# feixue94/sfd2

Hardware: AMD Instinct MI355X
Metric: images/sec extract+match (1600x1200, n4096) (higher is better)
Workload: dtype f16c

## Files before the change

### sfd2_amd/csrc/conv1x1_kernels.hip

```cpp
#include "sfd2_internal.h"
#include <stdlib.h>
#include <algorithm>

#define NT1 512
#define GPX 64
#define NST 4
#define STAGE_BYTES (GPX * 512)

typedef __attribute__((address_space(3))) void lds_void_t;
typedef const __attribute__((address_space(1))) void gbl_void_t;

__device__ __forceinline__ h4_t c1_cvt4(float a, float b, float c, float d)
{
    h4_t r;
    r[0] = (half_t)a; r[1] = (half_t)b; r[2] = (half_t)c; r[3] = (half_t)d;
    return r;
}

template <bool HAS_RES>
__global__ __launch_bounds__(NT1, 2)
void conv1x1_c256_kernel(const half_t *__restrict__ in, int npix, const half_t *__restrict__ w ,
                         const float *__restrict__ scale, const float *__restrict__ shift, int relu,
                         const half_t *__restrict__ res, half_t *__restrict__ out, int groups_per_block,
                         const half_t *__restrict__ zero_page )
{
    extern __shared__ __attribute__((aligned(16))) unsigned char smem[];
    unsigned char *Xs = smem;
    float *SS = reinterpret_cast<float *>(smem + NST * STAGE_BYTES);

    const int tid = threadIdx.x, lane = tid & 63;
    const int wave = __builtin_amdgcn_readfirstlane(tid >> 6);
    const int lrow = lane & 31, lhi = lane >> 5;
    const int cg = wave & 3, ph = wave >> 2;
    const int ngroups = (npix + GPX - 1) / GPX;
    const int g0 = blockIdx.x * groups_per_block;
    int g1 = g0 + groups_per_block;
    if (g1 > ngroups) g1 = ngroups;
    if (g0 >= g1) return;

    h8_t a[2][16];
#pragma unroll
    for (int t = 0; t < 2; ++t)
#pragma unroll
        for (int kk = 0; kk < 16; ++kk)
            a[t][kk] = *reinterpret_cast<const h8_t *>(w + (size_t)(cg * 64 + t * 32 + lrow) * 256 + kk * 16 + lhi * 8);
    for (int t = tid; t < 256; t += NT1) { SS[t] = scale[t]; SS[256 + t] = shift[t]; }

#define ISSUE_G(g_)                                                                                        \
    {                                                                                                      \
        unsigned char *st = Xs + ((g_) & (NST - 1)) * STAGE_BYTES;                                         \
        _Pragma("unroll") for (int i = 0; i < 4; ++i) {                                                    \
            const int ch = wave * 4 + i;                                                                   \
            const int p = ch * 2 + lhi;                                        \
            const long long gp = (long long)(g_)*GPX + p;                                                  \
            const half_t *src = gp < npix ? in + gp * 256 + ((lrow ^ (p & 31)) << 3) : zero_page + (lrow << 3); \
            __builtin_amdgcn_global_load_lds((gbl_void_t *)src, (lds_void_t *)(st + ch * 1024), 16, 0, 0); \
        }                                                                                                  \
    }
#define WAIT_GROUP()                                                                                       \
    asm volatile("s_waitcnt vmcnt(8) lgkmcnt(0)\n\ts_barrier" ::: "memory")

    ISSUE_G(g0)
    if (g0 + 1 < g1) { ISSUE_G(g0 + 1) }
    if (g0 + 2 < g1) { ISSUE_G(g0 + 2) }
    SFD2_BARRIER_DRAIN();

    for (int g = g0; g < g1; ++g) {
        if (g != g0) {
            if (g + 2 < g1) WAIT_GROUP(); else SFD2_BARRIER_DRAIN();
        }
        const unsigned char *st = Xs + (g & (NST - 1)) * STAGE_BYTES;
        const int p = ph * 32 + lrow;
        const long long gp = (long long)g * GPX + p;
        const bool inb = gp < npix;
        const size_t obase = (size_t)(inb ? gp : 0) * 256 + cg * 64;

        uint4 rq[2][2];
        if (HAS_RES) {
#pragma unroll
            for (int t = 0; t < 2; ++t)
#pragma unroll
                for (int m = 0; m < 2; ++m) {
                    rq[t][m] = make_uint4(0, 0, 0, 0);
                    if (inb) rq[t][m] = *reinterpret_cast<const uint4 *>(res + obase + t * 32 + 8 * (2 * m + lhi));
                }
            asm volatile("" ::: "memory");
        }
        if (g + 3 < g1) { ISSUE_G(g + 3) }

        f32x16_t acc[2];
#pragma unroll
        for (int t = 0; t < 2; ++t)
#pragma unroll
            for (int r = 0; r < 16; ++r) acc[t][r] = 0.0f;
        const unsigned char *xp = st + p * 512;
        const int sw = p & 31;
#pragma unroll
        for (int kk = 0; kk < 16; ++kk) {
            const h8_t b = *reinterpret_cast<const h8_t *>(xp + (((kk * 2 + lhi) ^ sw) << 4));
            acc[0] = __builtin_amdgcn_mfma_f32_32x32x16_f16(a[0][kk], b, acc[0], 0, 0, 0);
            acc[1] = __builtin_amdgcn_mfma_f32_32x32x16_f16(a[1][kk], b, acc[1], 0, 0, 0);
        }

#pragma unroll
        for (int t = 0; t < 2; ++t) {
            const int cl = cg * 64 + t * 32 + 4 * lhi;
#pragma unroll
            for (int m = 0; m < 2; ++m) {
                uint2 rp[2] = {make_uint2(0, 0), make_uint2(0, 0)};
                if (HAS_RES) {
                    const auto s0 = __builtin_amdgcn_permlane32_swap(rq[t][m].x, rq[t][m].z, false, false);
                    const auto s1 = __builtin_amdgcn_permlane32_swap(rq[t][m].y, rq[t][m].w, false, false);
                    rp[0] = make_uint2(s0[0], s1[0]);
                    rp[1] = make_uint2(s0[1], s1[1]);
                }
                uint2 pk[2];
#pragma unroll
                for (int j = 0; j < 2; ++j) {
                    const int q = 2 * m + j;
                    const float4 sc = sfd2_lds_f4(SS + cl + 8 * q);
                    const float4 sh = sfd2_lds_f4(SS + 256 + cl + 8 * q);
                    float v0 = acc[t][4 * q + 0] * sc.x + sh.x;
                    float v1 = acc[t][4 * q + 1] * sc.y + sh.y;
                    float v2 = acc[t][4 * q + 2] * sc.z + sh.z;
                    float v3 = acc[t][4 * q + 3] * sc.w + sh.w;
                    if (HAS_RES) {
                        h4_t r;
                        __builtin_memcpy(&r, &rp[j], 8);
                        v0 += (float)r[0]; v1 += (float)r[1]; v2 += (float)r[2]; v3 += (float)r[3];
                    }
                    if (relu) { v0 = fmaxf(v0, 0.0f); v1 = fmaxf(v1, 0.0f); v2 = fmaxf(v2, 0.0f); v3 = fmaxf(v3, 0.0f); }
                    const h4_t hv = c1_cvt4(v0, v1, v2, v3);
                    __builtin_memcpy(&pk[j], &hv, 8);
                }
                const auto t0 = __builtin_amdgcn_permlane32_swap(pk[0].x, pk[1].x, false, false);
                const auto t1 = __builtin_amdgcn_permlane32_swap(pk[0].y, pk[1].y, false, false);
                if (inb)
                    *reinterpret_cast<uint4 *>(out + obase + t * 32 + 8 * (2 * m + lhi)) = make_uint4(t0[0], t1[0], t0[1], t1[1]);
            }
        }
    }
#undef ISSUE_G
#undef WAIT_GROUP
}

void launch_conv1x1_c256(hipStream_t st, const half_t *in, int npix, const half_t *w_rowmajor, const float *scale,
                         const float *shift, int relu, const half_t *res, half_t *out, const half_t *zero_page)
{
    static bool attr_done = false;
    static int slots = 256;
    const size_t lds = (size_t)NST * STAGE_BYTES + 512 * sizeof(float);
    if (!attr_done) {
        (void)hipFuncSetAttribute(reinterpret_cast<const void *>(conv1x1_c256_kernel<true>), hipFuncAttributeMaxDynamicSharedMemorySize, (int)lds);
        (void)hipFuncSetAttribute(reinterpret_cast<const void *>(conv1x1_c256_kernel<false>), hipFuncAttributeMaxDynamicSharedMemorySize, (int)lds);
        int dev = 0, cus = 0;
        if (hipGetDevice(&dev) == hipSuccess &&
            hipDeviceGetAttribute(&cus, hipDeviceAttributeMultiprocessorCount, dev) == hipSuccess && cus > 0)
            slots = cus;
        attr_done = true;
    }
    const int ngroups = (npix + GPX - 1) / GPX;
    if (ngroups == 0) return;
    const int gpb = (ngroups + sfd2_slots(slots) - 1) / sfd2_slots(slots);
    const int grid = (ngroups + gpb - 1) / gpb;
    if (res) hipLaunchKernelGGL(conv1x1_c256_kernel<true>, dim3(grid), dim3(NT1), lds, st, in, npix, w_rowmajor, scale, shift, relu, res, out, gpb, zero_page);
    else hipLaunchKernelGGL(conv1x1_c256_kernel<false>, dim3(grid), dim3(NT1), lds, st, in, npix, w_rowmajor, scale, shift, relu, res, out, gpb, zero_page);
}

#define GPXC 32
#define STAGE_C (2 * GPXC * 512)

#ifndef SFD2_R1_VSCALE
#define SFD2_R1_VSCALE 4.0f
#endif
#ifndef SFD2_C256_R1_STAGES
#define SFD2_C256_R1_STAGES 4
#endif
#define STAGE_R1 (GPXC * 512 + GPXC * 256)
#ifndef SFD2_C256_STAGGER
#define SFD2_C256_STAGGER 0
#endif
#ifndef SFD2_C256_SPLIT_ACC
#define SFD2_C256_SPLIT_ACC 0
#endif
#ifdef SFD2_C256_TRACE
#include <stdio.h>
__device__ unsigned long long g_c256_cyc[2][6][4];
#define C256_CYC(k_) if (blockIdx.x == 3 && (wave == 0 || wave == 4) && lane == 0 && g - g0 >= 4 && g - g0 < 10) g_c256_cyc[wave == 4][g - g0 - 4][k_] = __builtin_readcyclecounter();
#else
#define C256_CYC(k_)
#endif
#ifdef SFD2_C256_ABL
#define C256_ABL SFD2_C256_ABL
#else
#define C256_ABL 0
#endif
template <bool HAS_RES, int IN_C, bool OUT_C>
__global__ __launch_bounds__(NT1, 2)
void conv1x1_c256_c_kernel(const half_t *__restrict__ in, const half_t *__restrict__ in_c, int npix,
                           const half_t *__restrict__ w , const half_t *__restrict__ wc ,
                           const float *__restrict__ scale, const float *__restrict__ shift, int relu,
                           const half_t *__restrict__ res, const half_t *__restrict__ res_c,
                           half_t *__restrict__ out, half_t *__restrict__ out_c, int groups_per_block,
                           const half_t *__restrict__ zero_page, int sa, unsigned int *__restrict__ range )
{
    constexpr int NSTC = IN_C == 2 ? SFD2_C256_R1_STAGES : NST;
    constexpr int STB = IN_C == 2 ? STAGE_R1 : STAGE_C;
    constexpr int AHEAD = NSTC - 1;
    constexpr int CPG = IN_C == 1 ? 4 : IN_C == 2 ? 3 : 2;
    extern __shared__ __attribute__((aligned(16))) unsigned char smem[];
    unsigned char *Xs = smem;
    float *SS = reinterpret_cast<float *>(smem + NSTC * STB);

    const int tid = threadIdx.x, lane = tid & 63;
    const int wave = __builtin_amdgcn_readfirstlane(tid >> 6);
    const int lrow = lane & 31, lhi = lane >> 5;
    const int ngroups = (npix + GPXC - 1) / GPXC;
#ifdef SFD2_C256_INTERLEAVE
    const int g0 = 0;
    const int g1 = ((int)blockIdx.x < ngroups) ? (ngroups - (int)blockIdx.x + (int)gridDim.x - 1) / (int)gridDim.x : 0;
#define GRP(g_) ((int)blockIdx.x + (g_) * (int)gridDim.x)
#else
    const int g0 = blockIdx.x * groups_per_block;
    int g1 = g0 + groups_per_block;
    if (g1 > ngroups) g1 = ngroups;
#define GRP(g_) (g_)
#endif
    if (g0 >= g1) return;

    h8_t ah[16];
    v8i_t ac[8];
    {
        const size_t fo = ((size_t)wave * 8 * 64 + lane) * 16;
#pragma unroll
        for (int c = 0; c < 8; ++c) {
            ah[2 * c] = *reinterpret_cast<const h8_t *>(w + fo + (size_t)c * 64 * 16);
            ah[2 * c + 1] = *reinterpret_cast<const h8_t *>(w + fo + (size_t)c * 64 * 16 + 8);
            ac[c] = sfd2_cat8(*reinterpret_cast<const h8_t *>(wc + fo + (size_t)c * 64 * 16), *reinterpret_cast<const h8_t *>(wc + fo + (size_t)c * 64 * 16 + 8));
        }
    }
    for (int t = tid; t < 256; t += NT1) { SS[t] = scale[t]; SS[256 + t] = shift[t]; }

#define ISSUE_GC(g_)                                                                                       \
    {                                                                                                      \
        unsigned char *st = Xs + (unsigned)((g_) - g0) % (unsigned)NSTC * STB;                             \
        _Pragma("unroll") for (int i = 0; i < 2; ++i) {                                                    \
            const int ch = wave * 2 + i;                                                                   \
            const int p = ch * 2 + lhi;                                                                    \
            const long long gp = (long long)GRP(g_)*GPXC + p;                                                 \
            const size_t so = (size_t)gp * 256 + ((lrow ^ (p & 31)) << 3);                                 \
            const half_t *s0 = gp < npix ? in + so : zero_page + (lrow << 3);                              \
            __builtin_amdgcn_global_load_lds((gbl_void_t *)s0, (lds_void_t *)(st + ch * 1024), 16, 0, 0);  \
            if (IN_C == 1) {                                                                               \
                const half_t *s1 = gp < npix ? in_c + so : zero_page + (lrow << 3);                        \
                __builtin_amdgcn_global_load_lds((gbl_void_t *)s1, (lds_void_t *)(st + GPXC * 512 + ch * 1024), 16, 0, 0); \
            }                                                                                              \
        }                                                                                                  \
        if (IN_C == 2) {    \
            const int p = wave * 4 + (lane >> 4);                                                          \
            const long long gp = (long long)GRP(g_)*GPXC + p;                                                 \
            const unsigned char *s1 = gp < npix ? reinterpret_cast<const unsigned char *>(in_c) + (size_t)gp * 256 + (((lane & 15) ^ (p & 15)) << 4) \
                                                : reinterpret_cast<const unsigned char *>(zero_page) + ((lane & 15) << 4); \
            __builtin_amdgcn_global_load_lds((gbl_void_t *)s1, (lds_void_t *)(st + GPXC * 512 + wave * 1024), 16, 0, 0); \
        }                                                                                                  \
    }
#define WAIT_GROUP_C()                                                                                     \
                        \
    asm volatile("s_waitcnt vmcnt(%0) lgkmcnt(0)\n\ts_barrier" ::"n"((AHEAD - 1) * CPG) : "memory")

#pragma unroll
    for (int a = 0; a < AHEAD; ++a)
        if (g0 + a < g1) { ISSUE_GC(g0 + a) }
    SFD2_BARRIER_DRAIN();

    float mx = 0.0f;
    constexpr bool STG = SFD2_C256_STAGGER != 0;
    const int grp = wave >> 2;
    if (STG && grp == 1) asm volatile("s_barrier" ::: "memory");
    for (int g = g0; g < g1; ++g) {
        C256_CYC(0)
        if (!STG && g != g0) {
            if (g + AHEAD - 1 < g1) WAIT_GROUP_C(); else SFD2_BARRIER_DRAIN();
        }
        C256_CYC(1)
        const unsigned char *st = Xs + (unsigned)(g - g0) % (unsigned)NSTC * STB;
        const int p = lrow;
        const long long gp = (long long)GRP(g) * GPXC + p;
        const bool inb = gp < npix;
        const size_t obase = (size_t)(inb ? gp : 0) * 256 + wave * 32;

        uint4 rq[2], rc[2];
        if (HAS_RES) {
#pragma unroll
            for (int m = 0; m < 2; ++m) {
                rq[m] = make_uint4(0, 0, 0, 0);
                rc[m] = make_uint4(0, 0, 0, 0);
                if (inb) {
                    rq[m] = *reinterpret_cast<const uint4 *>(res + obase + 8 * (2 * m + lhi));
                    rc[m] = *reinterpret_cast<const uint4 *>(res_c + obase + 8 * (2 * m + lhi));
                }
            }
            asm volatile("" ::: "memory");
        }
        if (!(C256_ABL & 2) && g + AHEAD < g1) { ISSUE_GC(g + AHEAD) }

        f32x16_t acc;
#pragma unroll
        for (int r = 0; r < 16; ++r) acc[r] = 0.0f;
        const unsigned char *xp = st + p * 512;
        const int sw = p & 31;
        f32x16_t acl;
        if (!IN_C) {
#pragma unroll
            for (int r = 0; r < 16; ++r) acl[r] = 0.0f;
        }
        if (IN_C == 2) {
#if SFD2_C256_SPLIT_ACC
            f32x16_t acs;
#pragma unroll
            for (int r = 0; r < 16; ++r) acs[r] = 0.0f;
#endif
            const unsigned char *xr = st + GPXC * 512 + p * 256 + 8 * lhi;
            const int sr = p & 15;
#pragma unroll
            for (int c = 0; c < 8; ++c) {
                const h8_t b0 = *reinterpret_cast<const h8_t *>(xp + (((c * 4 + lhi) ^ sw) << 4));
                const h8_t b1 = *reinterpret_cast<const h8_t *>(xp + (((c * 4 + 2 + lhi) ^ sw) << 4));
                const h4_t r0h = *reinterpret_cast<const h4_t *>(xr + (((2 * c) ^ sr) << 4)), r1h = *reinterpret_cast<const h4_t *>(xr + (((2 * c + 1) ^ sr) << 4));
                uint2 r0, r1;
                __builtin_memcpy(&r0, &r0h, 8);
                __builtin_memcpy(&r1, &r1h, 8);
                acc = __builtin_amdgcn_mfma_f32_32x32x16_f16(ah[2 * c], b0, acc, 0, 0, 0);
                acc = __builtin_amdgcn_mfma_f32_32x32x16_f16(ah[2 * c + 1], b1, acc, 0, 0, 0);
                typedef short s2v_t __attribute__((ext_vector_type(2)));
                v8i_t bu;
#pragma unroll
                for (int h = 0; h < 2; ++h) {
                    const h8_t bb = h ? b1 : b0;
                    const uint2 rr = h ? r1 : r0;
#pragma unroll
                    for (int q = 0; q < 2; ++q) {
                        s2v_t v = {0, 0};
                        v = __builtin_amdgcn_cvt_scalef32_pk_fp8_f16(v, h2_t{bb[4 * q], bb[4 * q + 1]}, SFD2_R1_VSCALE, false);
                        v = __builtin_amdgcn_cvt_scalef32_pk_fp8_f16(v, h2_t{bb[4 * q + 2], bb[4 * q + 3]}, SFD2_R1_VSCALE, true);
                        unsigned int vb;
                        __builtin_memcpy(&vb, &v, 4);
                        bu[2 * h + q] = (int)(q ? rr.y : rr.x);
                        bu[4 + 2 * h + q] = (int)vb;
                    }
                }
#if SFD2_C256_SPLIT_ACC
                acs = __builtin_amdgcn_mfma_scale_f32_32x32x64_f8f6f4(ac[c], bu, acs, 0, 0, 0, sa, 0, 0x7f7f7f7f);
#else
                acc = __builtin_amdgcn_mfma_scale_f32_32x32x64_f8f6f4(ac[c], bu, acc, 0, 0, 0, sa, 0, 0x7f7f7f7f);
#endif
            }
#if SFD2_C256_SPLIT_ACC
            asm volatile("" : "+v"(acs));
#pragma unroll
            for (int r = 0; r < 16; ++r) acc[r] += acs[r];
#endif
            asm volatile("" : "+v"(acc));
        } else
#pragma unroll
        for (int kk = 0; kk < 16; ++kk) {
            const h8_t b = *reinterpret_cast<const h8_t *>(xp + (((kk * 2 + lhi) ^ sw) << 4));
            acc = __builtin_amdgcn_mfma_f32_32x32x16_f16(ah[kk], b, acc, 0, 0, 0);
            if (!IN_C) acl = __builtin_amdgcn_mfma_f32_32x32x16_f16(sfd2_half8(ac[kk >> 1], kk & 1), b, acl, 0, 0, 0);
        }
        if (IN_C == 2) {
        } else if (IN_C) {
#pragma unroll
            for (int c = 0; c < 8; ++c) {
                const v8i_t b = sfd2_cat8(*reinterpret_cast<const h8_t *>(xp + GPXC * 512 + (((c * 4 + lhi) ^ sw) << 4)),
                                          *reinterpret_cast<const h8_t *>(xp + GPXC * 512 + (((c * 4 + 2 + lhi) ^ sw) << 4)));
                acc = __builtin_amdgcn_mfma_scale_f32_32x32x64_f8f6f4(ac[c], b, acc, 0, 0, 0, sa, 0, 0x7f7f7f7f);
            }
            asm volatile("" : "+v"(acc));
        } else {
#pragma unroll
            for (int r = 0; r < 16; ++r) acc[r] = __builtin_fmaf(acl[r], 1.0f / 2048.0f, acc[r]);
        }

        asm volatile("" : "+v"(acc));
        C256_CYC(2)
        if (STG) {
            asm volatile("" : "+v"(acc));
            if (g + AHEAD < g1) asm volatile("s_waitcnt vmcnt(%0) lgkmcnt(0)" ::"n"((AHEAD - 1) * CPG) : "memory");
            else asm volatile("s_waitcnt vmcnt(0) lgkmcnt(0)" ::: "memory");
            __builtin_amdgcn_sched_barrier(0);
            asm volatile("s_barrier" ::: "memory");
            __builtin_amdgcn_sched_barrier(0);
        }
        const int cl = wave * 32 + 4 * lhi;
#pragma unroll
        for (int m = 0; m < 2; ++m) {
            uint2 rp[2] = {make_uint2(0, 0), make_uint2(0, 0)}, rcp[2] = {make_uint2(0, 0), make_uint2(0, 0)};
            if (HAS_RES) {
                const auto s0 = __builtin_amdgcn_permlane32_swap(rq[m].x, rq[m].z, false, false);
                const auto s1 = __builtin_amdgcn_permlane32_swap(rq[m].y, rq[m].w, false, false);
                rp[0] = make_uint2(s0[0], s1[0]);
                rp[1] = make_uint2(s0[1], s1[1]);
                const auto c0 = __builtin_amdgcn_permlane32_swap(rc[m].x, rc[m].z, false, false);
                const auto c1 = __builtin_amdgcn_permlane32_swap(rc[m].y, rc[m].w, false, false);
                rcp[0] = make_uint2(c0[0], c1[0]);
                rcp[1] = make_uint2(c0[1], c1[1]);
            }
            uint2 pk[2], ck[2];
#pragma unroll
            for (int j = 0; j < 2; ++j) {
                const int q = 2 * m + j;
                const float4 sc = sfd2_lds_f4(SS + cl + 8 * q);
                const float4 sh = sfd2_lds_f4(SS + 256 + cl + 8 * q);
                float4 ad = make_float4(0.f, 0.f, 0.f, 0.f);
                if (HAS_RES) {
                    h4_t r;
                    __builtin_memcpy(&r, &rp[j], 8);
                    ad = make_float4((float)r[0] + sfd2_corr_lo(rcp[j].x, 0), (float)r[1] + sfd2_corr_lo(rcp[j].x, 1),
                                     (float)r[2] + sfd2_corr_lo(rcp[j].y, 0), (float)r[3] + sfd2_corr_lo(rcp[j].y, 1));
                }
                sfd2_epi4<HAS_RES>(acc[4 * q + 0], acc[4 * q + 1], acc[4 * q + 2], acc[4 * q + 3], sc, sh, ad, relu ? 0.0f : -SFD2_C_SAT, pk[j], ck[j], mx, inb);
            }
            const auto t0 = __builtin_amdgcn_permlane32_swap(pk[0].x, pk[1].x, false, false);
            const auto t1 = __builtin_amdgcn_permlane32_swap(pk[0].y, pk[1].y, false, false);
            if (inb && (!(C256_ABL & 1) || t0[0] == 0x12345678u)) *reinterpret_cast<uint4 *>(out + obase + 8 * (2 * m + lhi)) = make_uint4(t0[0], t1[0], t0[1], t1[1]);
            if (OUT_C) {
                const auto u0 = __builtin_amdgcn_permlane32_swap(ck[0].x, ck[1].x, false, false);
                const auto u1 = __builtin_amdgcn_permlane32_swap(ck[0].y, ck[1].y, false, false);
                if (inb) *reinterpret_cast<uint4 *>(out_c + obase + 8 * (2 * m + lhi)) = make_uint4(u0[0], u1[0], u0[1], u1[1]);
            }
        }
        C256_CYC(3)
        if (STG && !(grp == 1 && g + 1 == g1)) {
            __builtin_amdgcn_sched_barrier(0);
            asm volatile("s_waitcnt lgkmcnt(0)\n\ts_barrier" ::: "memory");
            __builtin_amdgcn_sched_barrier(0);
        }
    }
    sfd2_range_commit(range, sfd2_wave_max_bits(mx));
#undef ISSUE_GC
#undef GRP
#undef WAIT_GROUP_C
}

template <int RES, bool OUT_F32, bool OUT_PLANES>
__global__ __launch_bounds__(NT1, 2)
void conv1x1_c256_x3_kernel(const half_t *__restrict__ in, const half_t *__restrict__ in_lo, int npix,
                            const half_t *__restrict__ w, const half_t *__restrict__ wl,
                            const float *__restrict__ scale, const float *__restrict__ shift, int relu,
                            const void *res_v, const half_t *res_lo, float *__restrict__ out, half_t *out_hi, half_t *out_lo,
                            int groups_per_block, const half_t *__restrict__ zero_page)
{
    constexpr bool HAS_RES = RES != 0;
    const float *res = static_cast<const float *>(res_v);
    const half_t *res_hi = static_cast<const half_t *>(res_v);
    extern __shared__ __attribute__((aligned(16))) unsigned char smem[];
    unsigned char *Xs = smem;
    float *SS = reinterpret_cast<float *>(smem + NST * STAGE_C);

    const int tid = threadIdx.x, lane = tid & 63;
    const int wave = __builtin_amdgcn_readfirstlane(tid >> 6);
    const int lrow = lane & 31, lhi = lane >> 5;
    const int ngroups = (npix + GPXC - 1) / GPXC;
    const int g0 = blockIdx.x * groups_per_block;
    int g1 = g0 + groups_per_block;
    if (g1 > ngroups) g1 = ngroups;
    if (g0 >= g1) return;

    h8_t ah[16];
    v8i_t al[8];
    {
        const size_t fo = ((size_t)wave * 8 * 64 + lane) * 16;
#pragma unroll
        for (int c = 0; c < 8; ++c) {
            ah[2 * c] = *reinterpret_cast<const h8_t *>(w + fo + (size_t)c * 64 * 16);
            ah[2 * c + 1] = *reinterpret_cast<const h8_t *>(w + fo + (size_t)c * 64 * 16 + 8);
            al[c] = sfd2_cat8(*reinterpret_cast<const h8_t *>(wl + fo + (size_t)c * 64 * 16), *reinterpret_cast<const h8_t *>(wl + fo + (size_t)c * 64 * 16 + 8));
        }
    }
    for (int t = tid; t < 256; t += NT1) { SS[t] = scale[t]; SS[256 + t] = shift[t]; }

#define ISSUE_GX(g_)                                                                                       \
    {                                                                                                      \
        unsigned char *st = Xs + ((g_) & (NST - 1)) * STAGE_C;                                             \
        _Pragma("unroll") for (int i = 0; i < 2; ++i) {                                                    \
            const int ch = wave * 2 + i;                                                                   \
            const int p = ch * 2 + lhi;                                                                    \
            const long long gp = (long long)(g_)*GPXC + p;                                                 \
            const size_t so = (size_t)gp * 256 + ((lrow ^ (p & 31)) << 3);                                 \
            const half_t *s0 = gp < npix ? in + so : zero_page + (lrow << 3);                              \
            const half_t *s1 = gp < npix ? in_lo + so : zero_page + (lrow << 3);                           \
            __builtin_amdgcn_global_load_lds((gbl_void_t *)s0, (lds_void_t *)(st + ch * 1024), 16, 0, 0);  \
            __builtin_amdgcn_global_load_lds((gbl_void_t *)s1, (lds_void_t *)(st + GPXC * 512 + ch * 1024), 16, 0, 0); \
        }                                                                                                  \
    }
#define WAIT_GROUP_X()                                                                                     \
                              \
    asm volatile("s_waitcnt vmcnt(8) lgkmcnt(0)\n\ts_barrier" ::: "memory")

    ISSUE_GX(g0)
    if (g0 + 1 < g1) { ISSUE_GX(g0 + 1) }
    if (g0 + 2 < g1) { ISSUE_GX(g0 + 2) }
    SFD2_BARRIER_DRAIN();

    for (int g = g0; g < g1; ++g) {
        if (g != g0) {
            if (g + 2 < g1) WAIT_GROUP_X(); else SFD2_BARRIER_DRAIN();
        }
        const unsigned char *st = Xs + (g & (NST - 1)) * STAGE_C;
        const int p = lrow;
        const long long gp = (long long)g * GPXC + p;
        const bool inb = gp < npix;
        const size_t obase = (size_t)(inb ? gp : 0) * 256 + wave * 32 + 4 * lhi;

        float4 rr[4];
        uint4 rh16[2], rl16[2];
        if (RES == 1) {
#pragma unroll
            for (int q = 0; q < 4; ++q) rr[q] = *reinterpret_cast<const float4 *>(res + obase + 8 * q);
            asm volatile("" ::: "memory");
        }
        if (RES == 2) {
#pragma unroll
            for (int m = 0; m < 2; ++m) {
                const size_t o16 = (size_t)(inb ? gp : 0) * 256 + wave * 32 + 8 * (2 * m + lhi);
                rh16[m] = *reinterpret_cast<const uint4 *>(res_hi + o16);
                rl16[m] = *reinterpret_cast<const uint4 *>(res_lo + o16);
            }
            asm volatile("" ::: "memory");
        }
        if (g + 3 < g1) { ISSUE_GX(g + 3) }

        f32x16_t acc, acl;
#pragma unroll
        for (int r = 0; r < 16; ++r) { acc[r] = 0.0f; acl[r] = 0.0f; }
        const unsigned char *xp = st + p * 512;
        const int sw = p & 31;
#pragma unroll
        for (int kk = 0; kk < 16; ++kk) {
            const h8_t b = *reinterpret_cast<const h8_t *>(xp + (((kk * 2 + lhi) ^ sw) << 4));
            const h8_t bl = *reinterpret_cast<const h8_t *>(xp + GPXC * 512 + (((kk * 2 + lhi) ^ sw) << 4));
            acc = __builtin_amdgcn_mfma_f32_32x32x16_f16(ah[kk], b, acc, 0, 0, 0);
            acl = __builtin_amdgcn_mfma_f32_32x32x16_f16(ah[kk], bl, acl, 0, 0, 0);
            acl = __builtin_amdgcn_mfma_f32_32x32x16_f16(sfd2_half8(al[kk >> 1], kk & 1), b, acl, 0, 0, 0);
        }
        const int cl = wave * 32 + 4 * lhi;
        h4_t rh[4], rl[4];
        if (RES == 2) {
#pragma unroll
            for (int m = 0; m < 2; ++m) {
                const auto a0 = __builtin_amdgcn_permlane32_swap(rh16[m].x, rh16[m].z, false, false);
                const auto a1 = __builtin_amdgcn_permlane32_swap(rh16[m].y, rh16[m].w, false, false);
                const auto b0 = __builtin_amdgcn_permlane32_swap(rl16[m].x, rl16[m].z, false, false);
                const auto b1 = __builtin_amdgcn_permlane32_swap(rl16[m].y, rl16[m].w, false, false);
                const uint2 h0 = make_uint2(a0[0], a1[0]), h1 = make_uint2(a0[1], a1[1]), l0 = make_uint2(b0[0], b1[0]), l1 = make_uint2(b0[1], b1[1]);
                __builtin_memcpy(&rh[2 * m], &h0, 8); __builtin_memcpy(&rh[2 * m + 1], &h1, 8);
                __builtin_memcpy(&rl[2 * m], &l0, 8); __builtin_memcpy(&rl[2 * m + 1], &l1, 8);
            }
        }
        uint2 ph[4], pl[4];
#pragma unroll
        for (int q = 0; q < 4; ++q) {
            const float4 sc = sfd2_lds_f4(SS + cl + 8 * q);
            const float4 sh = sfd2_lds_f4(SS + 256 + cl + 8 * q);
            float v0 = (acc[4 * q + 0] + acl[4 * q + 0] * (1.0f / 2048.0f)) * sc.x + sh.x;
            float v1 = (acc[4 * q + 1] + acl[4 * q + 1] * (1.0f / 2048.0f)) * sc.y + sh.y;
            float v2 = (acc[4 * q + 2] + acl[4 * q + 2] * (1.0f / 2048.0f)) * sc.z + sh.z;
            float v3 = (acc[4 * q + 3] + acl[4 * q + 3] * (1.0f / 2048.0f)) * sc.w + sh.w;
            if (RES == 2) {
                rr[q] = make_float4((float)rh[q][0] + (float)rl[q][0] * (1.0f / 2048.0f), (float)rh[q][1] + (float)rl[q][1] * (1.0f / 2048.0f),
                                    (float)rh[q][2] + (float)rl[q][2] * (1.0f / 2048.0f), (float)rh[q][3] + (float)rl[q][3] * (1.0f / 2048.0f));
            }
            if (HAS_RES) { v0 += rr[q].x; v1 += rr[q].y; v2 += rr[q].z; v3 += rr[q].w; }
            if (relu) { v0 = fmaxf(v0, 0.0f); v1 = fmaxf(v1, 0.0f); v2 = fmaxf(v2, 0.0f); v3 = fmaxf(v3, 0.0f); }
            if (OUT_F32 && inb) *reinterpret_cast<float4 *>(out + obase + 8 * q) = make_float4(v0, v1, v2, v3);
            if (OUT_PLANES) {
                h4_t hv = {(half_t)v0, (half_t)v1, (half_t)v2, (half_t)v3};
                h4_t lv = {(half_t)((v0 - (float)hv[0]) * 2048.0f), (half_t)((v1 - (float)hv[1]) * 2048.0f),
                           (half_t)((v2 - (float)hv[2]) * 2048.0f), (half_t)((v3 - (float)hv[3]) * 2048.0f)};
                __builtin_memcpy(&ph[q], &hv, 8);
                __builtin_memcpy(&pl[q], &lv, 8);
            }
        }
        if (OUT_PLANES) {
#pragma unroll
            for (int m = 0; m < 2; ++m) {
                const auto t0 = __builtin_amdgcn_permlane32_swap(ph[2 * m].x, ph[2 * m + 1].x, false, false);
                const auto t1 = __builtin_amdgcn_permlane32_swap(ph[2 * m].y, ph[2 * m + 1].y, false, false);
                const auto u0 = __builtin_amdgcn_permlane32_swap(pl[2 * m].x, pl[2 * m + 1].x, false, false);
                const auto u1 = __builtin_amdgcn_permlane32_swap(pl[2 * m].y, pl[2 * m + 1].y, false, false);
                const size_t o16 = (size_t)(inb ? gp : 0) * 256 + wave * 32 + 8 * (2 * m + lhi);
                if (inb) {
                    *reinterpret_cast<uint4 *>(out_hi + o16) = make_uint4(t0[0], t1[0], t0[1], t1[1]);
                    *reinterpret_cast<uint4 *>(out_lo + o16) = make_uint4(u0[0], u1[0], u0[1], u1[1]);
                }
            }
        }
    }
#undef ISSUE_GX
#undef WAIT_GROUP_X
}

void launch_conv1x1_c256_x3(hipStream_t st, const half_t *in, const half_t *in_lo, int npix, const half_t *w, const half_t *wl,
                            const float *scale, const float *shift, int relu, const void *res, const half_t *res_lo, float *out, half_t *out_hi,
                            half_t *out_lo, const half_t *zero_page)
{
    static bool attr_done = false;
    static int slots = 256;
    const size_t lds = (size_t)NST * STAGE_C + 512 * sizeof(float);
    if (!attr_done) {
#define C256X_ATTR(...) (void)hipFuncSetAttribute(reinterpret_cast<const void *>(conv1x1_c256_x3_kernel<__VA_ARGS__>), hipFuncAttributeMaxDynamicSharedMemorySize, (int)lds);
        C256X_ATTR(0, true, false) C256X_ATTR(0, false, true) C256X_ATTR(1, true, false) C256X_ATTR(1, true, true) C256X_ATTR(2, false, true) C256X_ATTR(2, true, true)
#undef C256X_ATTR
        int dev = 0, cus = 0;
        if (hipGetDevice(&dev) == hipSuccess && hipDeviceGetAttribute(&cus, hipDeviceAttributeMultiprocessorCount, dev) == hipSuccess && cus > 0)
            slots = cus;
        attr_done = true;
    }
    const int ngroups = (npix + GPXC - 1) / GPXC;
    if (ngroups == 0) return;
    const int gpb = (ngroups + sfd2_slots(slots) - 1) / sfd2_slots(slots);
    const int grid = (ngroups + gpb - 1) / gpb;
#define C256X_GO(...) hipLaunchKernelGGL((conv1x1_c256_x3_kernel<__VA_ARGS__>), dim3(grid), dim3(NT1), lds, st, in, in_lo, npix, w, wl, scale, shift, relu, res, res_lo, out, out_hi, out_lo, gpb, zero_page)
    const int rmode = !res ? 0 : (res_lo ? 2 : 1);
    if (rmode == 0 && out && !out_hi) C256X_GO(0, true, false);
    else if (rmode == 0 && !out && out_hi) C256X_GO(0, false, true);
    else if (rmode == 1 && out && !out_hi) C256X_GO(1, true, false);
    else if (rmode == 1 && out && out_hi) C256X_GO(1, true, true);
    else if (rmode == 2 && !out && out_hi) C256X_GO(2, false, true);
    else if (rmode == 2 && out && out_hi) C256X_GO(2, true, true);
    else abort();
#undef C256X_GO
}

void launch_conv1x1_c256_c(hipStream_t st, const half_t *in, const half_t *in_c, int npix, const half_t *w_frag,
                           const half_t *wc_frag, const float *scale, const float *shift, int relu, const half_t *res,
                           const half_t *res_c, half_t *out, half_t *out_c, const half_t *zero_page, int sbyte, unsigned int *range, Rec rin, Rec rout)
{
    static bool attr_done = false;
    static int slots = 256;
    const size_t lds = rin == Rec::Resid8 ? (size_t)SFD2_C256_R1_STAGES * STAGE_R1 + 512 * sizeof(float) : (size_t)NST * STAGE_C + 512 * sizeof(float);
    if (!attr_done) {
        const size_t lds_max = std::max((size_t)SFD2_C256_R1_STAGES * STAGE_R1, (size_t)NST * STAGE_C) + 512 * sizeof(float);
#define C256C_ATTR(R_, I_, O_) (void)hipFuncSetAttribute(reinterpret_cast<const void *>(conv1x1_c256_c_kernel<R_, I_, O_>), hipFuncAttributeMaxDynamicSharedMemorySize, (int)lds_max);
        C256C_ATTR(true, 1, true) C256C_ATTR(false, 1, true) C256C_ATTR(false, 1, false) C256C_ATTR(true, 0, true) C256C_ATTR(false, 2, false)
#undef C256C_ATTR
        int dev = 0, cus = 0;
        if (hipGetDevice(&dev) == hipSuccess &&
            hipDeviceGetAttribute(&cus, hipDeviceAttributeMultiprocessorCount, dev) == hipSuccess && cus > 0)
            slots = cus;
        attr_done = true;
    }
    const int ngroups = (npix + GPXC - 1) / GPXC;
    if (ngroups == 0) return;
    const int gpb = (ngroups + sfd2_slots(slots) - 1) / sfd2_slots(slots);
    const int grid = (ngroups + gpb - 1) / gpb;
    const int sa = (sbyte & 255) * 0x01010101;
#define C256C_GO(R_, I_, O_) hipLaunchKernelGGL((conv1x1_c256_c_kernel<R_, I_, O_>), dim3(grid), dim3(NT1), lds, st, in, in_c, npix, w_frag, wc_frag, scale, shift, relu, res, res_c, out, out_c, gpb, zero_page, sa, range)
    if (rin == Rec::Resid8) { if (rout == Rec::None && !res) C256C_GO(false, 2, false); else abort(); }
#ifdef SFD2_C256_TRACE
    if (rin == Rec::Resid8) {
        static int dumps = 0;
        if (npix > 100000 && ++dumps == 40) {
            (void)hipStreamSynchronize(st);
            static unsigned long long hc[2][6][4];
            (void)hipMemcpyFromSymbol(hc, HIP_SYMBOL(g_c256_cyc), sizeof(hc));
            for (int w = 0; w < 2; ++w)
                for (int t = 0; t < 6; ++t)
                    fprintf(stderr, "c256 trace wave %d group %d: wait+barrier %lld  reads+MFMAs %lld  epilogue %lld  to next top %lld\n", w * 4, t + 4,
                            (long long)(hc[w][t][1] - hc[w][t][0]), (long long)(hc[w][t][2] - hc[w][t][1]), (long long)(hc[w][t][3] - hc[w][t][2]),
                            t < 5 ? (long long)(hc[w][t + 1][0] - hc[w][t][3]) : 0ll);
        }
    }
#endif
    else if (rin == Rec::Unit8 && rout == Rec::Unit8) { if (res) C256C_GO(true, 1, true); else C256C_GO(false, 1, true); }
    else if (rin == Rec::Unit8 && rout == Rec::None && !res) C256C_GO(false, 1, false);
    else if (rin == Rec::None && rout == Rec::Unit8 && res) C256C_GO(true, 0, true);
    else abort();
#undef C256C_GO
}
```

Baseline: 716.7.

## Precompute FP8 value plane one group ahead into a double-buffered LDS slab

In the residual-8 path of the c256 1x1 conv kernel, the FP8 conversion of the f16 high part moves out of the inner MFMA loop. Each thread now converts one slot of the next group's record into a separate double-buffered LDS value plane while the current group's MFMAs run, and the inner loop just loads the prepared FP8 words. The in-flight wait depth shrinks by one group to make room for this lookahead, and LDS use grows by two value planes. The scale changes from a fixed VSCALE to 1/SFD2_C_XH_SCALE, and the unused stagger code path is removed.

```diff
diff --git a/sfd2_amd/csrc/conv1x1_kernels.hip b/sfd2_amd/csrc/conv1x1_kernels.hip
--- a/sfd2_amd/csrc/conv1x1_kernels.hip
+++ b/sfd2_amd/csrc/conv1x1_kernels.hip
@@ -170,16 +170,11 @@
 #define GPXC 32
 #define STAGE_C (2 * GPXC * 512)
 
-#ifndef SFD2_R1_VSCALE
-#define SFD2_R1_VSCALE 4.0f
-#endif
 #ifndef SFD2_C256_R1_STAGES
 #define SFD2_C256_R1_STAGES 4
 #endif
 #define STAGE_R1 (GPXC * 512 + GPXC * 256)
-#ifndef SFD2_C256_STAGGER
-#define SFD2_C256_STAGGER 0
-#endif
+#define VPLANE_R1 (GPXC * 256)
 #ifndef SFD2_C256_SPLIT_ACC
 #define SFD2_C256_SPLIT_ACC 0
 #endif
@@ -195,6 +190,42 @@
 #else
 #define C256_ABL 0
 #endif
+__device__ __forceinline__ void sfd2_r1_hi_pair(const unsigned char *hrec , int p, int v, h8_t &a, h8_t &b)
+{
+    const int s = 4 * (v >> 1) + (v & 1);
+    a = *reinterpret_cast<const h8_t *>(hrec + ((s ^ (p & 31)) << 4));
+    b = *reinterpret_cast<const h8_t *>(hrec + (((s + 2) ^ (p & 31)) << 4));
+}
+__device__ __forceinline__ v4i_t sfd2_r1_values(h8_t a, h8_t b)
+{
+    typedef short s2v_t __attribute__((ext_vector_type(2)));
+    v4i_t o;
+#pragma unroll
+    for (int h = 0; h < 2; ++h) {
+        const h8_t x = h ? b : a;
+#pragma unroll
+        for (int q = 0; q < 2; ++q) {
+            s2v_t w = {0, 0};
+            w = __builtin_amdgcn_cvt_scalef32_pk_fp8_f16(w, h2_t{x[4 * q], x[4 * q + 1]}, 1.0f / SFD2_C_XH_SCALE, false);
+            w = __builtin_amdgcn_cvt_scalef32_pk_fp8_f16(w, h2_t{x[4 * q + 2], x[4 * q + 3]}, 1.0f / SFD2_C_XH_SCALE, true);
+            int d;
+            __builtin_memcpy(&d, &w, 4);
+            o[2 * h + q] = d;
+        }
+    }
+    return o;
+}
+__device__ __forceinline__ void sfd2_r1_store_slot(v4i_t o, int p, int v, unsigned int vrec )
+{
+    asm volatile("ds_write_b128 %0, %1" ::"v"(vrec + ((unsigned)(v ^ (p & 15)) << 4)), "v"(o) : "memory");
+}
+__device__ __forceinline__ void sfd2_r1_value_slot(const unsigned char *hrec, int p, int v, unsigned int vrec)
+{
+    h8_t a, b;
+    sfd2_r1_hi_pair(hrec, p, v, a, b);
+    sfd2_r1_store_slot(sfd2_r1_values(a, b), p, v, vrec);
+}
+
 template <bool HAS_RES, int IN_C, bool OUT_C>
 __global__ __launch_bounds__(NT1, 2)
 void conv1x1_c256_c_kernel(const half_t *__restrict__ in, const half_t *__restrict__ in_c, int npix,
@@ -208,9 +239,12 @@
     constexpr int STB = IN_C == 2 ? STAGE_R1 : STAGE_C;
     constexpr int AHEAD = NSTC - 1;
     constexpr int CPG = IN_C == 1 ? 4 : IN_C == 2 ? 3 : 2;
+    constexpr int FLY = IN_C == 2 ? AHEAD - 2 : AHEAD - 1;
+    static_assert(FLY >= 1, "ring too shallow");
     extern __shared__ __attribute__((aligned(16))) unsigned char smem[];
     unsigned char *Xs = smem;
-    float *SS = reinterpret_cast<float *>(smem + NSTC * STB);
+    unsigned char *Vs = smem + NSTC * STB;
+    float *SS = reinterpret_cast<float *>(smem + NSTC * STB + (IN_C == 2 ? 2 * VPLANE_R1 : 0));
 
     const int tid = threadIdx.x, lane = tid & 63;
     const int wave = __builtin_amdgcn_readfirstlane(tid >> 6);
@@ -265,21 +299,24 @@
         }                                                                                                  \
     }
 #define WAIT_GROUP_C()                                                                                     \
-                        \
-    asm volatile("s_waitcnt vmcnt(%0) lgkmcnt(0)\n\ts_barrier" ::"n"((AHEAD - 1) * CPG) : "memory")
+                              \
+    asm volatile("s_waitcnt vmcnt(%0) lgkmcnt(0)\n\ts_barrier" ::"n"(FLY * CPG) : "memory")
+#define HREC_GC(g_) (Xs + (unsigned)((g_) - g0) % (unsigned)NSTC * STB + (tid & 31) * 512)
+#define VREC_GC(g_) ((unsigned)(size_t)(lds_void_t *)(Vs + ((g_) - g0) % 2 * VPLANE_R1) + (tid & 31) * 256)
 
 #pragma unroll
     for (int a = 0; a < AHEAD; ++a)
         if (g0 + a < g1) { ISSUE_GC(g0 + a) }
     SFD2_BARRIER_DRAIN();
+    if (IN_C == 2) {
+        sfd2_r1_value_slot(HREC_GC(g0), tid & 31, tid >> 5, VREC_GC(g0));
+        asm volatile("s_waitcnt lgkmcnt(0)\n\ts_barrier" ::: "memory");
+    }
 
     float mx = 0.0f;
-    constexpr bool STG = SFD2_C256_STAGGER != 0;
-    const int grp = wave >> 2;
-    if (STG && grp == 1) asm volatile("s_barrier" ::: "memory");
     for (int g = g0; g < g1; ++g) {
         C256_CYC(0)
-        if (!STG && g != g0) {
+        if (g != g0) {
             if (g + AHEAD - 1 < g1) WAIT_GROUP_C(); else SFD2_BARRIER_DRAIN();
         }
         C256_CYC(1)
@@ -303,6 +340,8 @@
             asm volatile("" ::: "memory");
         }
         if (!(C256_ABL & 2) && g + AHEAD < g1) { ISSUE_GC(g + AHEAD) }
+        h8_t nva, nvb;
+        if (IN_C == 2) sfd2_r1_hi_pair(HREC_GC(g + 1), tid & 31, tid >> 5, nva, nvb);
 
         f32x16_t acc;
 #pragma unroll
@@ -321,34 +360,22 @@
             for (int r = 0; r < 16; ++r) acs[r] = 0.0f;
 #endif
             const unsigned char *xr = st + GPXC * 512 + p * 256 + 8 * lhi;
+            const unsigned char *xv = Vs + (g - g0) % 2 * VPLANE_R1 + p * 256;
             const int sr = p & 15;
 #pragma unroll
             for (int c = 0; c < 8; ++c) {
                 const h8_t b0 = *reinterpret_cast<const h8_t *>(xp + (((c * 4 + lhi) ^ sw) << 4));
                 const h8_t b1 = *reinterpret_cast<const h8_t *>(xp + (((c * 4 + 2 + lhi) ^ sw) << 4));
                 const h4_t r0h = *reinterpret_cast<const h4_t *>(xr + (((2 * c) ^ sr) << 4)), r1h = *reinterpret_cast<const h4_t *>(xr + (((2 * c + 1) ^ sr) << 4));
+                const h8_t vh = *reinterpret_cast<const h8_t *>(xv + (((2 * c + lhi) ^ sr) << 4));
+                acc = __builtin_amdgcn_mfma_f32_32x32x16_f16(ah[2 * c], b0, acc, 0, 0, 0);
+                acc = __builtin_amdgcn_mfma_f32_32x32x16_f16(ah[2 * c + 1], b1, acc, 0, 0, 0);
                 uint2 r0, r1;
                 __builtin_memcpy(&r0, &r0h, 8);
                 __builtin_memcpy(&r1, &r1h, 8);
-                acc = __builtin_amdgcn_mfma_f32_32x32x16_f16(ah[2 * c], b0, acc, 0, 0, 0);
-                acc = __builtin_amdgcn_mfma_f32_32x32x16_f16(ah[2 * c + 1], b1, acc, 0, 0, 0);
-                typedef short s2v_t __attribute__((ext_vector_type(2)));
-                v8i_t bu;
-#pragma unroll
-                for (int h = 0; h < 2; ++h) {
-                    const h8_t bb = h ? b1 : b0;
-                    const uint2 rr = h ? r1 : r0;
-#pragma unroll
-                    for (int q = 0; q < 2; ++q) {
-                        s2v_t v = {0, 0};
-                        v = __builtin_amdgcn_cvt_scalef32_pk_fp8_f16(v, h2_t{bb[4 * q], bb[4 * q + 1]}, SFD2_R1_VSCALE, false);
-                        v = __builtin_amdgcn_cvt_scalef32_pk_fp8_f16(v, h2_t{bb[4 * q + 2], bb[4 * q + 3]}, SFD2_R1_VSCALE, true);
-                        unsigned int vb;
-                        __builtin_memcpy(&vb, &v, 4);
-                        bu[2 * h + q] = (int)(q ? rr.y : rr.x);
-                        bu[4 + 2 * h + q] = (int)vb;
-                    }
-                }
+                v4i_t vv;
+                __builtin_memcpy(&vv, &vh, 16);
+                const v8i_t bu = {(int)r0.x, (int)r0.y, (int)r1.x, (int)r1.y, vv[0], vv[1], vv[2], vv[3]};
 #if SFD2_C256_SPLIT_ACC
                 acs = __builtin_amdgcn_mfma_scale_f32_32x32x64_f8f6f4(ac[c], bu, acs, 0, 0, 0, sa, 0, 0x7f7f7f7f);
 #else
@@ -361,6 +388,8 @@
             for (int r = 0; r < 16; ++r) acc[r] += acs[r];
 #endif
             asm volatile("" : "+v"(acc));
+            const v4i_t nv = sfd2_r1_values(nva, nvb);
+            if (g + 1 < g1) sfd2_r1_store_slot(nv, tid & 31, tid >> 5, VREC_GC(g + 1));
         } else
 #pragma unroll
         for (int kk = 0; kk < 16; ++kk) {
@@ -384,14 +413,6 @@
 
         asm volatile("" : "+v"(acc));
         C256_CYC(2)
-        if (STG) {
-            asm volatile("" : "+v"(acc));
-            if (g + AHEAD < g1) asm volatile("s_waitcnt vmcnt(%0) lgkmcnt(0)" ::"n"((AHEAD - 1) * CPG) : "memory");
-            else asm volatile("s_waitcnt vmcnt(0) lgkmcnt(0)" ::: "memory");
-            __builtin_amdgcn_sched_barrier(0);
-            asm volatile("s_barrier" ::: "memory");
-            __builtin_amdgcn_sched_barrier(0);
-        }
         const int cl = wave * 32 + 4 * lhi;
 #pragma unroll
         for (int m = 0; m < 2; ++m) {
@@ -431,16 +452,13 @@
             }
         }
         C256_CYC(3)
-        if (STG && !(grp == 1 && g + 1 == g1)) {
-            __builtin_amdgcn_sched_barrier(0);
-            asm volatile("s_waitcnt lgkmcnt(0)\n\ts_barrier" ::: "memory");
-            __builtin_amdgcn_sched_barrier(0);
-        }
     }
     sfd2_range_commit(range, sfd2_wave_max_bits(mx));
 #undef ISSUE_GC
 #undef GRP
 #undef WAIT_GROUP_C
+#undef HREC_GC
+#undef VREC_GC
 }
 
 template <int RES, bool OUT_F32, bool OUT_PLANES>
@@ -639,9 +657,10 @@
 {
     static bool attr_done = false;
     static int slots = 256;
-    const size_t lds = rin == Rec::Resid8 ? (size_t)SFD2_C256_R1_STAGES * STAGE_R1 + 512 * sizeof(float) : (size_t)NST * STAGE_C + 512 * sizeof(float);
+    const size_t lds_r1 = (size_t)SFD2_C256_R1_STAGES * STAGE_R1 + 2 * VPLANE_R1;
+    const size_t lds = rin == Rec::Resid8 ? lds_r1 + 512 * sizeof(float) : (size_t)NST * STAGE_C + 512 * sizeof(float);
     if (!attr_done) {
-        const size_t lds_max = std::max((size_t)SFD2_C256_R1_STAGES * STAGE_R1, (size_t)NST * STAGE_C) + 512 * sizeof(float);
+        const size_t lds_max = std::max(lds_r1, (size_t)NST * STAGE_C) + 512 * sizeof(float);
 #define C256C_ATTR(R_, I_, O_) (void)hipFuncSetAttribute(reinterpret_cast<const void *>(conv1x1_c256_c_kernel<R_, I_, O_>), hipFuncAttributeMaxDynamicSharedMemorySize, (int)lds_max);
         C256C_ATTR(true, 1, true) C256C_ATTR(false, 1, true) C256C_ATTR(false, 1, false) C256C_ATTR(true, 0, true) C256C_ATTR(false, 2, false)
 #undef C256C_ATTR
```

Measured after the change: 719.3, median of 6. About the same (+0.4%).
